# wischmcj/pyQSM

Measured on AMD Instinct MI355X. Metric: Mpoints/s DBSCAN (1M-pt synthetic forest, eps=0.1, min_neighbors=10), higher is better.
Workload: dtype f64; 1 GPU; 1000000-point synthetic tree cloud (configs[1]), DBSCAN eps=0.1 min_neighbors=10, 20 clusters; replicas at N>1; points_per_gpu=1000000, parallelism=replicas x1

## Files before the change

### pyqsm_amd/csrc/dbscan.hip

```cpp
#include "grid.hpp"

#include <atomic>
#include <chrono>
#include <optional>
#include <vector>

namespace pyqsm {

static constexpr int kNoRoot = 0x7FFFFFFF;

__device__ __forceinline__ double sqdist(double ax, double ay, double az, double bx, double by,
                                         double bz) {
  double t0 = ax - bx, t1 = ay - by, t2 = az - bz;
  double d = t0 * t0;
  d = d + t1 * t1;
  d = d + t2 * t2;
  return d;
}


#define FOR_STENCIL(c, st, dir, q, body)                           \
  for (int dz__ = -1; dz__ <= 1; ++dz__)                           \
    for (int dy__ = -1; dy__ <= 1; ++dy__) {                       \
      const int row__ = (c) + dy__ * (st).nx + dz__ * (st).nxy;    \
// ... 75 lines not shown
          const int q = base + lane;
          const int m = qe - base < 64 ? qe - base : 64;
          if (q < qe) co.get(q, L.x[w][lane], L.y[w][lane], L.z[w][lane]);
          __builtin_amdgcn_wave_barrier();
          staged += m;
          if (mine)
            for (int j = 0; j < m; ++j)
              cnt += sqdist(x, y, z, L.x[w][j], L.y[w][j], L.z[w][j]) <= r2;
          __builtin_amdgcn_wave_barrier();
        }
      }
    }
  } else {
#pragma unroll
    for (int ri = 0; ri < 9; ++ri) {
      const int r = kRunOrder[ri];
      for (int base = t.qb[r]; base < t.qe[r] && !deferred; base += 64) {
        const int q = base + lane;
        const int m = t.qe[r] - base < 64 ? t.qe[r] - base : 64;
        if (q < t.qe[r]) co.get(q, L.x[w][lane], L.y[w][lane], L.z[w][lane]);
        __builtin_amdgcn_wave_barrier();
        staged += m;
#pragma unroll 4
        for (int j = 0; j < m; ++j)
          cnt += sqdist(x, y, z, L.x[w][j], L.y[w][j], L.z[w][j]) <= r2;
        __builtin_amdgcn_wave_barrier();
        const unsigned long long und = __ballot(live && cnt < min_pts);
        ++chunks;
        if ((__popcll(und) <= kStragglers || chunks >= max_chunks) &&
            !(ri == 8 && base + 64 >= t.qe[r])) {
          if (und != 0) {
            int slot = 0;
            const int lead = __ffsll(und) - 1;
            const int seg = blockIdx.x % kRestSegs;
            if (lane == lead) slot = atomicAdd(rest_cnt + seg, __popcll(und));
            slot = __shfl(slot, lead, 64);
            if (live && cnt < min_pts) {
              rest[size_t(seg) * seg_cap + slot + __popcll(und & ((1ull << lane) - 1ull))] = p;
              cnt = -1;
            }
          }
          deferred = true;
          break;
        }
      }
    }
  }
  if (live && cnt >= 0) {
    core[p] = cnt >= min_pts;
    co.mark_core(p, cnt >= min_pts);
  }
  if (live) {
    parent[p] = p;
    min_orig[p] = 0x7F7F7F7F;
    flag[p] = 0;
    if (p == n - 1) flag[n] = 0;
  }
  if (tests && lane == 0) atomicAdd(tests + (blockIdx.x & 255), static_cast<unsigned long long>(staged));
  });
}

struct Runs9 {
  int qb[9];
  int pre[10];
  __device__ __forceinline__ int at(int g) const {
    int q = qb[0] + g;
#pragma unroll
    for (int r = 1; r < 9; ++r) q = g >= pre[r] ? qb[r] + (g - pre[r]) : q;
    return q;
  }
};
static constexpr int kRunBatch = 3;
__device__ __forceinline__ int lane_bound(bool act, int c, int j, Stencil st, const CellDir& dir) {
  const int r = int((0x862071534ull >> (4 * (j >> 1))) & 15ull);
  const int cell = c + (r % 3 - 1) * st.nx + (r / 3 - 1) * st.nxy + ((j & 1) ? 2 : -1);
  int b = 0;
  if (act) {
    const DirWord w = dir.words[cell >> 5];
    b = dir.slots[CellDir::slot_of(w, cell)];
  }
  return b;
}
__device__ __forceinline__ Runs9 runs_of_lanes(int bound, int k) {
  Runs9 t;
  t.pre[0] = 0;
#pragma unroll
  for (int r = 0; r < 9; ++r) {
    t.qb[r] = __builtin_amdgcn_readlane(bound, 18 * k + 2 * r);
    t.pre[r + 1] = t.pre[r] + (__builtin_amdgcn_readlane(bound, 18 * k + 2 * r + 1) - t.qb[r]);
  }
  return t;
}

template <class CO>
__global__ __launch_bounds__(256) void k_core_rest(const int32_t* __restrict__ rest,
                                                   const int32_t* __restrict__ rest_cnt ,
                                                   int seg_cap, const GridPlan* __restrict__ plan,
                                                   const DirWord* __restrict__ dwords,
                                                   const int32_t* __restrict__ dslots,
                                                   const int32_t* __restrict__ cell_of, CO co, double r2,
                                                   int min_pts, uint8_t* __restrict__ core,
    unsigned long long* __restrict__ st ) {
  stamped(st, [&] {
  const CellDir dir{dwords, dslots};
  if (!plan->ok) return;
  const Stencil st = plan_stencil(plan);
  const int lane = threadIdx.x & 63;
  const int mine = rest_cnt[lane];
  int incl = mine;
#pragma unroll
  for (int off = 1; off < 64; off <<= 1) {
    const int v = __shfl_up(incl, off, 64);
    if (lane >= off) incl += v;
  }
  const int m = __shfl(incl, 63, 64);
  const int grp = lane / 18, j = lane % 18;
  for (int i0 = (blockIdx.x * 4 + (threadIdx.x >> 6)) * kRunBatch; i0 < m; i0 += gridDim.x * 4 * kRunBatch) {
    int p = 0;
#pragma unroll
    for (int k = 0; k < kRunBatch; ++k) {
      if (i0 + k >= m) break;
      const int seg = __popcll(__ballot(incl <= i0 + k));
      const int before = __shfl(incl - mine, seg, 64);
      const int pk = rest[size_t(seg) * seg_cap + (i0 + k - before)];
      p = grp == k ? pk : p;
    }
    const bool act = grp < kRunBatch && i0 + grp < m;
    double x = 0.0, y = 0.0, z = 0.0;
    int c = 0;
    if (act) {
      co.get(p, x, y, z);
      c = cell_of[p];
    }
    const int bound = lane_bound(act, c, j, st, dir);
#pragma unroll
    for (int k = 0; k < kRunBatch; ++k) {
      if (i0 + k >= m) break;
      const Runs9 t = runs_of_lanes(bound, k);
      const int pk = __builtin_amdgcn_readlane(p, 18 * k);
      const double xk = __shfl(x, 18 * k, 64), yk = __shfl(y, 18 * k, 64), zk = __shfl(z, 18 * k, 64);
      int cnt = 0;
      for (int g0 = 0; g0 < t.pre[9] && cnt < min_pts; g0 += 64) {
        const int g = g0 + lane;
        const bool hit = g < t.pre[9] && co.d2(t.at(g), xk, yk, zk) <= r2;
        cnt += __popcll(__ballot(hit));
      }
      if (lane == 0) {
        core[pk] = cnt >= min_pts;
        co.mark_core(pk, cnt >= min_pts);
      }
    }
  }
  });
}


__device__ __forceinline__ int ld_parent(const int* parent, int i) {
  return __hip_atomic_load(parent + i, __ATOMIC_RELAXED, __HIP_MEMORY_SCOPE_AGENT);
}
__device__ __forceinline__ void st_parent(int* parent, int i, int v) {
  __hip_atomic_store(parent + i, v, __ATOMIC_RELAXED, __HIP_MEMORY_SCOPE_AGENT);
}

__device__ __forceinline__ unsigned link_prio(int x) { return unsigned(x) * 0x9E3779B1u; }

__device__ __forceinline__ int find_root(int* parent, int x) {
  int cur = ld_parent(parent, x);
  if (cur != x) {
    int prev = x, next;
    while (cur != (next = ld_parent(parent, cur))) {
      st_parent(parent, prev, next);
      prev = cur;
      cur = next;
    }
  }
  return cur;
}

__device__ __forceinline__ void unite(int* parent, int a, int b) {
  int ra = find_root(parent, a), rb = find_root(parent, b);
  while (ra != rb) {
    if (link_prio(ra) < link_prio(rb)) {
      int t = ra;
      ra = rb;
      rb = t;
    }
    const int old = atomicCAS(parent + ra, ra, rb);
    if (old == ra) break;
    ra = find_root(parent, old);
    rb = find_root(parent, rb);
  }
}


__global__ __launch_bounds__(1024) void k_sub_rep(int n, const int32_t* __restrict__ sub_of,
                                                 const uint8_t* __restrict__ core,
                                                 const int32_t* __restrict__ order,
                                                 int* __restrict__ parent,
                                                 const int32_t* __restrict__ cell_of,
                                                 int4* __restrict__ rec,
                                                 int* __restrict__ run_min,
                                                 int4* __restrict__ list,
                                                 int32_t* __restrict__ list_cnt, const GridPlan* __restrict__ plan,
                                                 int4* __restrict__ list_xyz,
    unsigned long long* __restrict__ st ) {
  stamped(st, [&] {
  if (!plan->ok) return;
  const int nx = plan->nx, ny = plan->ny;
  const int lane = threadIdx.x & 63, w = threadIdx.x >> 6;
  const int base = blockIdx.x * 1024 + w * 64;
  const int p = base + lane;
  const bool live = p < n;
  int sid = 0, s = n, e = n, ord = 0x7FFFFFFF, cell = 0;
  bool c = false;
  const bool c_prev = base >= 64 && p - 64 < n && core[p - 64];
  const bool c_next = p + 64 < n && core[p + 64];
  const int o_next = c_next ? order[p + 64] : 0x7FFFFFFF;
  if (live) {
    sid = sub_of[p];
    c = core[p];
    if (c) ord = order[p];
    cell = cell_of[p];
    const int2 run = *reinterpret_cast<const int2*>(rec + sid);
    s = run.x;
    e = run.x + run.y;
  }
  const unsigned long long cb = __ballot(c);
  int lead = -1;
  const int s0 = __shfl(s, 0, 64);
  if (s0 < base && s0 >= base - 64) {
    const unsigned long long f = __ballot(c_prev && base - 64 + lane >= s0);
    if (f) lead = base - 64 + __ffsll(f) - 1;
  } else {
    for (int q0 = s0; q0 < base; q0 += 64) {
      const int q = q0 + lane;
      const unsigned long long f = __ballot(q < base && core[q]);
      if (f) {
        lead = q0 + __ffsll(f) - 1;
        break;
      }
    }
  }
  int rep = -1;
  if (c) {
    if (s < base && lead >= 0) {
      rep = lead;
    } else {
      const int lo = s > base ? s - base : 0;
      rep = base + __ffsll(cb & (~0ull << lo)) - 1;
    }
    parent[p] = rep;
  }
  const bool is_rep = c && rep == p;
  int mn = ord;
  const int seg_end = e - base < 64 ? e - base : 64;
#pragma unroll
  for (int off = 1; off < 64; off <<= 1) {
    const int o = __shfl_down(mn, off, 64);
    if (lane + off < seg_end) mn = o < mn ? o : mn;
  }
  const unsigned long long tail = __ballot(is_rep && e > base + 64);
  if (tail) {
    const int t = __ffsll(tail) - 1;
    const int et = __shfl(e, t, 64);
    int m2 = base + 64 + lane < et ? o_next : 0x7FFFFFFF;
    for (int q = base + 128 + lane; q < et; q += 64)
      if (core[q]) m2 = min(m2, order[q]);
#pragma unroll
    for (int off = 32; off > 0; off >>= 1) {
      const int o = __shfl_xor(m2, off, 64);
      m2 = o < m2 ? o : m2;
    }
    if (lane == t) mn = min(mn, m2);
  }
  if (is_rep) {
    rec[sid].z = rep;
    run_min[rep] = mn;
  }
  __shared__ int wcount[16], wbase[16];
  const unsigned long long b = __ballot(is_rep);
  if (lane == 0) wcount[w] = __popcll(b);
  __syncthreads();
  if (threadIdx.x == 0) {
    int tot = 0;
    for (int k = 0; k < 16; ++k) tot += wcount[k];
    int base2 = tot ? atomicAdd(list_cnt, tot) : 0;
    for (int k = 0; k < 16; ++k) {
      wbase[k] = base2;
      base2 += wcount[k];
    }
  }
  __syncthreads();
  if (is_rep) {
    const int slot = wbase[w] + __popcll(b & ((1ull << lane) - 1ull));
    const int c1 = cell;
    list[slot] = make_int4(rep, c1, sid, e - rep);
    list_xyz[slot] = make_int4(c1 % nx, (c1 / nx) % ny, c1 / (nx * ny), sid & 7);
  }
  });
}

__constant__ signed char kSubOffsets[62][3] = {{1,0,0}, {-1,1,0}, {0,1,0}, {1,1,0}, {-1,-1,1}, {0,-1,1}, {1,-1,1}, {-1,0,1}, {0,0,1}, {1,0,1}, {-1,1,1}, {0,1,1}, {1,1,1}, {2,0,0}, {-2,1,0}, {2,1,0}, {-2,2,0}, {-1,2,0}, {0,2,0}, {1,2,0}, {2,2,0}, {-2,-2,1}, {-1,-2,1}, {0,-2,1}, {1,-2,1}, {2,-2,1}, {-2,-1,1}, {2,-1,1}, {-2,0,1}, {2,0,1}, {-2,1,1}, {2,1,1}, {-2,2,1}, {-1,2,1}, {0,2,1}, {1,2,1}, {2,2,1}, {-2,-2,2}, {-1,-2,2}, {0,-2,2}, {1,-2,2}, {2,-2,2}, {-2,-1,2}, {-1,-1,2}, {0,-1,2}, {1,-1,2}, {2,-1,2}, {-2,0,2}, {-1,0,2}, {0,0,2}, {1,0,2}, {2,0,2}, {-2,1,2}, {-1,1,2}, {0,1,2}, {1,1,2}, {2,1,2}, {-2,2,2}, {-1,2,2}, {0,2,2}, {1,2,2}, {2,2,2}};

__global__ __launch_bounds__(256) void k_flatten_reps(const int4* __restrict__ list,
                                                      const int32_t* __restrict__ m_ptr,
                                                      int* __restrict__ parent, int max_steps,
                                                      int4* __restrict__ rec ) {
  const int m = *m_ptr;
  int s = blockIdx.x * 256 + threadIdx.x;
  if (s >= m) return;
  const int4 me = list[s];
  const int p = me.x;
  int r = p, steps = 0;
  for (int nx = parent[r]; nx != r && steps < max_steps; nx = parent[r], ++steps) r = nx;
  parent[p] = r;
  if (rec) {
    int* const word = reinterpret_cast<int*>(rec + (me.z & ~7)) + 3;
    const int old = atomicCAS(word, 0, r + 1);
    if (old != 0 && old != r + 1 && old != -1) *word = -1;
  }
}

static constexpr int kSubPerWave = 4;

struct SubNbr {
  int q0, n2, rep;
};
__device__ __forceinline__ SubNbr sub_neighbour(bool active, const int4 at, int dx, int dy, int dz, int nx, int ny,
                                                const CellDir& dir, const int4* __restrict__ rec) {
  const int gx = 2 * (at.x - 1) + (at.w & 1) - dx, gy = 2 * (at.y - 1) + ((at.w >> 1) & 1) - dy,
            gz = 2 * (at.z - 1) + ((at.w >> 2) & 1) - dz;
  const int c2 = (((gz >> 1) + 1) * ny + ((gy >> 1) + 1)) * nx + ((gx >> 1) + 1);
  const int oct = (gx & 1) | ((gy & 1) << 1) | ((gz & 1) << 2);
  SubNbr out{0, 0, -1};
  DirWord w{0u, 0u};
  if (active) w = dir.words[c2 >> 5];
  if ((w.bits >> (c2 & 31)) & 1u) {
    const int b2 = dir.slots[CellDir::slot_of(w, c2)];
    const int4 r = rec[b2 * 8 + oct];
    if (r.y > 0) {
      out.q0 = r.x;
      out.n2 = r.y;
      out.rep = r.z;
    }
  }
  return out;
}

template <class CO>
__global__ __launch_bounds__(256) void k_hook_sub(const int4* __restrict__ list,
                                                  const int4* __restrict__ list_xyz,
                                                  const int32_t* __restrict__ m_ptr,
                                                  const GridPlan* __restrict__ plan,
                                                  const DirWord* __restrict__ dwords,
                                                  const int32_t* __restrict__ dslots,
                                                  const int4* __restrict__ rec, CO co, double r2,
                                                  const uint8_t* __restrict__ core,
                                                  int* __restrict__ parent,
    unsigned long long* __restrict__ st ) {
  stamped(st, [&] {
  const CellDir dir{dwords, dslots};
  if (!plan->ok) return;
  const int nx = plan->nx, ny = plan->ny;
  const int m = *m_ptr;
  const int k = threadIdx.x & 63;
  const int t = k & 15, grp = k >> 4;
  const int o_dx = t < 13 ? kSubOffsets[t][0] : 0, o_dy = t < 13 ? kSubOffsets[t][1] : 0,
            o_dz = t < 13 ? kSubOffsets[t][2] : 0;
  for (int s0 = (blockIdx.x * 4 + (threadIdx.x >> 6)) * kSubPerWave; s0 < m; s0 += gridDim.x * 4 * kSubPerWave) {
    const bool live = s0 + grp < m;
    const int4 me = list[min(s0 + grp, m - 1)], at = list_xyz[min(s0 + grp, m - 1)];
    const SubNbr nb2 = sub_neighbour(live && t < 13, at, o_dx, o_dy, o_dz, nx, ny, dir, rec);
    const int p = me.x, n1 = me.w;
    unsigned todo = unsigned(__ballot(nb2.rep >= 0) >> (16 * grp)) & 0xFFFFu;
    int base = 0, hooked = -1;
    while (__ballot(todo != 0)) {
      const int src = (k & 48) + (todo ? __ffs(todo) - 1 : 0);
      const int qb = __shfl(nb2.q0, src, 64), nb = __shfl(nb2.n2, src, 64), rb = __shfl(nb2.rep, src, 64);
      const int sh = nb > 1 ? 32 - __clz(nb - 1) : 0;
      const int pairs = n1 << sh;
      const int idx = base + t;
      const int j = idx & ((1 << sh) - 1);
      bool hit = false;
      if (todo && idx < pairs && j < nb) hit = co.core_pair_within(p + (idx >> sh), qb + j, core, r2);
      const bool found = ((__ballot(hit) >> (16 * grp)) & 0xFFFFull) != 0;
      if (found) {
        hooked = rb;
        todo = 0;
      } else if (todo) {
        base += 16;
        if (base >= pairs) {
          todo &= todo - 1;
          base = 0;
        }
      }
    }
    if (hooked >= 0 && t == 0) parent[p] = parent[hooked];
  }
  });
}

template <class CO>
__device__ __forceinline__ bool wave_pair_within(const CO& co, int p, int n1, int qb, int nb, int k,
                                                 const uint8_t* __restrict__ core, double r2) {
  const int sh = nb > 1 ? 32 - __clz(nb - 1) : 0;
  const int pairs = n1 << sh;
  bool found = false;
  for (int base = 0; base < pairs && !found; base += 64) {
    const int idx = base + k;
    const int j = idx & ((1 << sh) - 1);
    bool hit = false;
    if (idx < pairs && j < nb) hit = co.core_pair_within(p + (idx >> sh), qb + j, core, r2);
    found = __ballot(hit) != 0;
  }
  return found;
}

template <class CO>
__device__ __forceinline__ void seam_unite(const int4 me, const int4 at, int k, int o_dx, int o_dy, int o_dz,
                                           int nx, int ny, const CellDir& dir,
                                           const int4* __restrict__ rec, const CO& co, double r2,
                                           const uint8_t* __restrict__ core, int* parent) {
  const SubNbr nb2 = sub_neighbour(k < 62, at, o_dx, o_dy, o_dz, nx, ny, dir, rec);
  const int p = me.x, n1 = me.w, rep2 = nb2.rep;
  const int* vparent = parent;
  int a1 = 0, a2 = 0;
  if (rep2 >= 0) {
    a1 = vparent[p];
    a2 = vparent[rep2];
  }
  bool need = rep2 >= 0 && !(a1 == a2 || a2 == p || a1 == rep2);
  int root2 = -1;
  if (need) {
    int ra = a1, rb = a2;
    for (;;) {
      const int pa = ld_parent(parent, ra), pb = ld_parent(parent, rb);
      if (pa == ra && pb == rb) break;
      ra = pa;
      rb = pb;
    }
    need = ra != rb;
    root2 = rb;
  }
  unsigned long long todo = __ballot(need);
  while (todo) {
    const int src = __ffsll(todo) - 1;
    todo &= todo - 1;
    const int qb = __shfl(nb2.q0, src, 64), nb = __shfl(nb2.n2, src, 64), rb = __shfl(rep2, src, 64);
    const int tree = __shfl(root2, src, 64);
    if (wave_pair_within(co, p, n1, qb, nb, k, core, r2)) {
      if (k == 0) unite(parent, p, rb);
      todo &= ~__ballot(root2 == tree);
    }
  }
}

template <class CO>
__global__ __launch_bounds__(256) void k_union_sub(const int4* __restrict__ list,
                                                   const int4* __restrict__ list_xyz,
                                                   const int32_t* __restrict__ m_ptr,
                                                   const GridPlan* __restrict__ plan,
                                                   const DirWord* __restrict__ dwords,
                                                   const int32_t* __restrict__ dslots,
                                                   const int4* __restrict__ rec, CO co, double r2,
                                                   const uint8_t* __restrict__ core, int* parent,
                                                   unsigned long long* __restrict__ seam_cnt ,
    unsigned long long* __restrict__ st ) {
  stamped(st, [&] {
  const CellDir dir{dwords, dslots};
  if (!plan->ok) return;
  const int nx = plan->nx, ny = plan->ny;
  const int m = *m_ptr;
  const int k = threadIdx.x & 63;
  const int t = k & 15, grp = k >> 4;
  const int o_dx = k < 62 ? kSubOffsets[k][0] : 0, o_dy = k < 62 ? kSubOffsets[k][1] : 0,
            o_dz = k < 62 ? kSubOffsets[k][2] : 0;
  const int c_off = t < 9 ? (t % 3 - 1) + (t / 3 - 1) * nx : 0;
  const int layer = nx * ny;
  for (int s0 = (blockIdx.x * 4 + (threadIdx.x >> 6)) * kSubPerWave; s0 < m; s0 += gridDim.x * 4 * kSubPerWave) {
    const bool live = s0 + grp < m;
    const int4 me = list[min(s0 + grp, m - 1)];
    const int* vparent = parent;
    const int r_s = vparent[me.x];
    const int c2 = me.y + c_off;
    int word[2] = {0, 0};
    DirWord dw[2] = {{0u, 0u}, {0u, 0u}};
    if (live && t < 9) {
#pragma unroll
      for (int l = 0; l < 2; ++l) dw[l] = dir.words[(c2 - l * layer) >> 5];
    }
    int b2[2] = {0, 0};
    bool occ[2];
#pragma unroll
    for (int l = 0; l < 2; ++l) {
      occ[l] = (dw[l].bits >> ((c2 - l * layer) & 31)) & 1u;
      if (occ[l]) b2[l] = dir.slots[CellDir::slot_of(dw[l], c2 - l * layer)];
    }
#pragma unroll
    for (int l = 0; l < 2; ++l)
      if (occ[l]) word[l] = rec[b2[l] * 8].w;
    const unsigned long long seams =
        __ballot((word[0] != 0 && word[0] != r_s + 1) || (word[1] != 0 && word[1] != r_s + 1));
    if (!seams) continue;
    for (int u = 0; u < kSubPerWave; ++u) {
      if (!((seams >> (16 * u)) & 0xFFFFull)) continue;
      if (seam_cnt && k == 0) atomicAdd(seam_cnt, 1ull);
      seam_unite(list[s0 + u], list_xyz[s0 + u], k, o_dx, o_dy, o_dz, nx, ny, dir, rec, co, r2, core, parent);
    }
  }
  });
}

template <class CO>
__global__ __launch_bounds__(256) void k_union_points(int n, Stencil st,
                                                      const DirWord* __restrict__ dwords,
                                                      const int32_t* __restrict__ dslots,
                                                      const int32_t* __restrict__ cell_of, CO co, double r2,
                                                      const uint8_t* __restrict__ core, int* parent) {
  const CellDir dir{dwords, dslots};
  int p = blockIdx.x * 256 + threadIdx.x;
  if (p >= n || !core[p]) return;
  double x, y, z;
  co.get(p, x, y, z);
  const int c = cell_of[p];
  const volatile int* vparent = parent;
  int rp = find_root(parent, p);
  FOR_STENCIL(c, st, dir, q, {
    if (q < p && core[q] && co.d2(q, x, y, z) <= r2) {
      if (vparent[q] != rp) {
        unite(parent, p, q);
        rp = find_root(parent, p);
      }
    }
  })
}

__global__ __launch_bounds__(256) void k_flatten(int n, const uint8_t* __restrict__ core,
                                                 int* __restrict__ parent, const GridPlan* __restrict__ plan) {
  int p = blockIdx.x * 256 + threadIdx.x;
  if (!plan->ok || p >= n || !core[p]) return;
  int r = p;
  for (int nx = parent[r]; nx != r; nx = parent[r]) r = nx;
  parent[p] = r;
}

template <int kThreads>
__device__ __forceinline__ void block_append(bool take, int value, int32_t* __restrict__ list,
                                             int32_t* __restrict__ cnt) {
  constexpr int kWaves = kThreads / 64;
  __shared__ int wcount[kWaves], wbase[kWaves];
  const unsigned long long b = __ballot(take);
  const int lane = threadIdx.x & 63, w = threadIdx.x >> 6;
  if (lane == 0) wcount[w] = __popcll(b);
  __syncthreads();
  if (threadIdx.x == 0) {
    int tot = 0;
    for (int k = 0; k < kWaves; ++k) tot += wcount[k];
    int base = tot ? atomicAdd(cnt, tot) : 0;
    for (int k = 0; k < kWaves; ++k) {
      wbase[k] = base;
      base += wcount[k];
    }
  }
  __syncthreads();
  if (take) list[wbase[w] + __popcll(b & ((1ull << lane) - 1ull))] = value;
}

static constexpr int kFlagsThreads = 256, kFlagsPer = 16, kFlagsPerBlock = kFlagsThreads * kFlagsPer;
__device__ __forceinline__ void flags_role(int b, int n, const uint8_t* __restrict__ core,
                                           int32_t* __restrict__ rest, int32_t* __restrict__ rest_cnt) {
  constexpr int kWaves = kFlagsThreads / 64;
  __shared__ int fcount[kWaves], fbase[kWaves];
  const int lane = threadIdx.x & 63, w = threadIdx.x >> 6;
  const int p0 = b * kFlagsPerBlock + threadIdx.x;
  unsigned take = 0;
#pragma unroll
  for (int k = 0; k < kFlagsPer; ++k) {
    const int p = p0 + k * kFlagsThreads;
    take |= unsigned(p < n && !core[p]) << k;
  }
  int mine = __popc(take);
#pragma unroll
  for (int off = 32; off > 0; off >>= 1) mine += __shfl_xor(mine, off, 64);
  if (lane == 0) fcount[w] = mine;
  __syncthreads();
  if (threadIdx.x == 0) {
    int tot = 0;
    for (int k = 0; k < kWaves; ++k) tot += fcount[k];
    int base = tot ? atomicAdd(rest_cnt, tot) : 0;
    for (int k = 0; k < kWaves; ++k) {
      fbase[k] = base;
      base += fcount[k];
    }
  }
  __syncthreads();
  int at = fbase[w];
#pragma unroll
  for (int k = 0; k < kFlagsPer; ++k) {
    const bool t = (take >> k) & 1u;
    const unsigned long long bal = __ballot(t);
    if (t) rest[at + __popcll(bal & ((1ull << lane) - 1ull))] = p0 + k * kFlagsThreads;
    at += __popcll(bal);
  }
}

__global__ __launch_bounds__(kFlagsThreads) void k_noncore_list(int n, const uint8_t* __restrict__ core,
                                                                int32_t* __restrict__ rest,
                                                                int32_t* __restrict__ rest_cnt,
                                                                const GridPlan* __restrict__ plan) {
  if (!plan->ok) return;
  flags_role(blockIdx.x, n, core, rest, rest_cnt);
}

__global__ __launch_bounds__(256) void k_point_min(int n, const uint8_t* __restrict__ core,
                                                   const int* __restrict__ parent,
                                                   const int32_t* __restrict__ order,
                                                   int* __restrict__ min_orig,
                                                   int32_t* __restrict__ roots,
                                                   int32_t* __restrict__ roots_cnt,
                                                   const GridPlan* __restrict__ plan) {
  int p = blockIdx.x * 256 + threadIdx.x;
  const bool is_c = plan->ok && p < n && core[p];
  if (is_c) atomicMin(min_orig + parent[p], order[p]);
  block_append<256>(is_c && parent[p] == p, p, roots, roots_cnt);
}

static constexpr int kRepRootThreads = kFlagsThreads;
static_assert(kRepRootThreads == 256, "gl, the grid of the representatives' blocks, is cut in 256s");
__global__ __launch_bounds__(kRepRootThreads) void k_rep_root(const int4* __restrict__ list,
                                                  const int32_t* __restrict__ m_ptr,
                                                  int* __restrict__ parent,
                                                  const int* __restrict__ run_min,
                                                  int* __restrict__ min_orig,
                                                  int32_t* __restrict__ roots,
                                                  int32_t* __restrict__ roots_cnt, int rep_blocks, int n,
                                                  const uint8_t* __restrict__ core, int32_t* __restrict__ rest,
                                                  int32_t* __restrict__ rest_cnt,
                                                  const GridPlan* __restrict__ plan) {
  if (int(blockIdx.x) >= rep_blocks) {
    if (plan->ok) flags_role(blockIdx.x - rep_blocks, n, core, rest, rest_cnt);
    return;
  }
  const int m = *m_ptr;
  int s = blockIdx.x * kRepRootThreads + threadIdx.x;
  const bool active = s < m;
  int p = -1, r = -1, v = 0x7FFFFFFF;
  if (active) {
    p = list[s].x;
    r = p;
    for (int nx = parent[r]; nx != r; nx = parent[r]) r = nx;
    if (r != p) parent[p] = r;
    v = run_min[p];
  }
  const volatile int* vmin = min_orig;
  const int lane = threadIdx.x & 63;
  unsigned long long rem = __ballot(active);
  while (rem) {
    const int lead = __ffsll(rem) - 1;
    const int r0 = __shfl(r, lead, 64);
    const bool mine = active && r == r0;
    int mn = mine ? v : 0x7FFFFFFF;
#pragma unroll
    for (int off = 32; off > 0; off >>= 1) {
      const int o = __shfl_xor(mn, off, 64);
      mn = o < mn ? o : mn;
    }
    if (lane == lead && mn < vmin[r0]) atomicMin(min_orig + r0, mn);
    rem &= ~__ballot(mine);
  }
  block_append<256>(active && r == p, p, roots, roots_cnt);
}

static constexpr int kRankCap = 4096;
static constexpr int kNumberThreads = 1024;

__global__ __launch_bounds__(kNumberThreads) void k_number(int n, const int32_t* __restrict__ roots,
                                                           const int32_t* __restrict__ roots_cnt,
                                                           int* __restrict__ min_orig,
                                                           uint32_t* __restrict__ bits ,
                                                           int32_t* __restrict__ wpre ,
                                                           int32_t* __restrict__ done ,
                                                           const GridPlan* __restrict__ plan,
    unsigned long long* __restrict__ st ) {
  stamped(st, [&] {
  if (!plan->ok) return;
  const int R = *roots_cnt;
  const int t = threadIdx.x;
  if (R <= kRankCap) {
    if (blockIdx.x != 0) return;
    __shared__ unsigned long long key[kRankCap];
    int P = 2;
    while (P < R) P <<= 1;
    for (int i = t; i < P; i += kNumberThreads) {
      unsigned long long k = ~0ull;
      if (i < R) {
        const int r = roots[i];
        k = (static_cast<unsigned long long>(min_orig[r]) << 32) | static_cast<uint32_t>(r);
      }
      key[i] = k;
    }
    __syncthreads();
    for (int k = 2; k <= P; k <<= 1)
      for (int j = k >> 1; j > 0; j >>= 1) {
        for (int i = t; i < P; i += kNumberThreads) {
          const int l = i ^ j;
          if (l > i) {
            const unsigned long long a = key[i], b = key[l];
            if ((a > b) == ((i & k) == 0)) {
              key[i] = b;
              key[l] = a;
            }
          }
        }
        __syncthreads();
      }
    for (int i = t; i < R; i += kNumberThreads) min_orig[static_cast<uint32_t>(key[i])] = i;
    return;
  }
  for (int i = blockIdx.x * kNumberThreads + t; i < R; i += gridDim.x * kNumberThreads) {
    const int v = min_orig[roots[i]];
    __hip_atomic_fetch_or(bits + (v >> 5), 1u << (v & 31), __ATOMIC_RELAXED, __HIP_MEMORY_SCOPE_AGENT);
  }
  __shared__ int last;
  __threadfence();
  __syncthreads();
  if (t == 0) last = atomicAdd(done, 1) == int(gridDim.x) - 1;
  __syncthreads();
  if (!last) return;
  __threadfence();
  __shared__ int wsum[kNumberThreads / 64];
  const int lane = t & 63, wv = t >> 6;
  const int nw = n / 32 + 1;
  int carry = 0;
  for (int w0 = 0; w0 < nw; w0 += 16 * kNumberThreads) {
    const int i0 = w0 + 16 * t;
    int cnt[16], sum = 0;
#pragma unroll
    for (int k = 0; k < 16; ++k) {
      cnt[k] = i0 + k < nw ? __popc(__hip_atomic_load(bits + i0 + k, __ATOMIC_RELAXED, __HIP_MEMORY_SCOPE_AGENT)) : 0;
      sum += cnt[k];
    }
    int incl = sum;
#pragma unroll
    for (int off = 1; off < 64; off <<= 1) {
      const int o = __shfl_up(incl, off, 64);
      if (lane >= off) incl += o;
    }
    if (lane == 63) wsum[wv] = incl;
    __syncthreads();
    int before = carry, total = 0;
    for (int k = 0; k < kNumberThreads / 64; ++k) {
      before += k < wv ? wsum[k] : 0;
      total += wsum[k];
    }
    int run = before + incl - sum;
#pragma unroll
    for (int k = 0; k < 16; ++k)
      if (i0 + k < nw) {
        wpre[i0 + k] = run;
        run += cnt[k];
      }
    carry += total;
    __syncthreads();
  }
  });
}

__device__ __forceinline__ int cluster_number(int v, int n_roots, const uint32_t* __restrict__ bits,
                                              const int32_t* __restrict__ wpre) {
  if (n_roots <= kRankCap) return v;
  return wpre[v >> 5] + __popc(bits[v >> 5] & ((1u << (v & 31)) - 1u));
}

static constexpr int kLabelThreads = 256;
template <class CO>
__global__ __launch_bounds__(kLabelThreads) void k_labels(int n, const int32_t* __restrict__ rest,
                                                          const int32_t* __restrict__ rest_cnt,
                                                          const GridPlan* __restrict__ plan,
                                                          const DirWord* __restrict__ dwords,
                                                          const int32_t* __restrict__ dslots,
                                                          const int32_t* __restrict__ cell_of, CO co, double r2,
                                                          const uint8_t* __restrict__ core,
                                                          const int* __restrict__ parent,
                                                          const int* __restrict__ min_orig,
                                                          const int32_t* __restrict__ roots_cnt,
                                                          const uint32_t* __restrict__ bits,
                                                          const int32_t* __restrict__ wpre,
                                                          const int32_t* __restrict__ order,
                                                          int64_t* __restrict__ labels,
                                                          uint8_t* __restrict__ is_core,
    unsigned long long* __restrict__ st ) {
  stamped(st, [&] {
  const CellDir dir{dwords, dslots};
  if (!plan->ok) return;
  constexpr int kWaves = kLabelThreads / 64;
  const int n_roots = *roots_cnt;
  const int lane = threadIdx.x & 63;
  {
    const int p = blockIdx.x * kLabelThreads + threadIdx.x;
    const bool is_c = p < n && core[p];
    if (is_c) {
      const int v = min_orig[parent[parent[p]]];
      labels[order[p]] = int64_t(cluster_number(v, n_roots, bits, wpre));
    }
    if (p < n && is_core) is_core[order[p]] = is_c;
  }
  const int m = *rest_cnt;
  const Stencil sten = plan_stencil(plan);
  const int first = (blockIdx.x * kWaves + __builtin_amdgcn_readfirstlane(threadIdx.x >> 6)) * kRunBatch;
  const int grp = lane / 18, j = lane % 18;
  for (int i0 = first; i0 < m; i0 += gridDim.x * kWaves * kRunBatch) {
    const bool act = grp < kRunBatch && i0 + grp < m;
    double x = 0.0, y = 0.0, z = 0.0;
    int p = 0, c = 0;
    if (act) {
      p = rest[i0 + grp];
      co.get(p, x, y, z);
      c = cell_of[p];
    }
    const int bound = lane_bound(act, c, j, sten, dir);
#pragma unroll
    for (int k = 0; k < kRunBatch; ++k) {
      if (i0 + k >= m) break;
      const Runs9 t = runs_of_lanes(bound, k);
      const int pk = __builtin_amdgcn_readlane(p, 18 * k);
      const double xk = __shfl(x, 18 * k, 64), yk = __shfl(y, 18 * k, 64), zk = __shfl(z, 18 * k, 64);
      int best = kNoRoot;
      for (int g0 = 0; g0 < t.pre[9]; g0 += 64) {
        const int g = g0 + lane;
        if (g < t.pre[9]) {
          const int q = t.at(g);
          if (core[q] && co.d2(q, xk, yk, zk) <= r2) {
            const int mo = min_orig[parent[parent[q]]];
            best = mo < best ? mo : best;
          }
        }
      }
#pragma unroll
      for (int off = 32; off > 0; off >>= 1) {
        const int o = __shfl_xor(best, off, 64);
        best = o < best ? o : best;
      }
      if (lane == 0)
        labels[order[pk]] = best == kNoRoot ? int64_t(-1) : int64_t(cluster_number(best, n_roots, bits, wpre));
    }
  }
  });
}

static int cluster_binned(Ctx* c, int64_t n, double eps, int32_t min_pts, bool radius_inclusive, const DevGrid& g,
                          const SubCells& sub, const GridPlan* d_plan, int64_t* labels, uint8_t* is_core,
                          const int32_t** count_out) {
  const bool fine = g.cell <= eps * (1.0 + 1.0 / 524288.0);
  const int N = int(n);
  const dim3 grid(ceil_div(n, 256)), block(256);
  const Stencil st{g.nx, g.nx * g.ny};
  const CellDir dir = cell_dir(g);
  const double r2 = radius_inclusive ? eps * eps : nextafter(eps * eps, 0.0);
  uint8_t* core;
  int *parent, *min_orig;
  int32_t* flag;
  PQ_TRY(c->arena.get(size_t(n), &core));
  PQ_TRY(c->arena.get(size_t(n), &parent));
  PQ_TRY(c->arena.get(size_t(n), &min_orig));
  PQ_TRY(c->arena.get(size_t(n) + 1, &flag));
  uint32_t* const bits = reinterpret_cast<uint32_t*>(flag);
  int32_t *roots, *wpre;
  PQ_TRY(c->arena.get(size_t(n), &roots));
  PQ_TRY(c->arena.get(size_t(n / 32) + 1, &wpre));
  int4* list;
  int32_t* list_cnt;
  int* run_min;
  PQ_TRY(c->arena.get(size_t(n), &run_min));
  PQ_TRY(c->arena.get(size_t(n), &list));
  int4* list_xyz;
  PQ_TRY(c->arena.get(size_t(n), &list_xyz));
  list_cnt = sub.zeroed4;
  int32_t* const roots_cnt = list_cnt + 1;
  int32_t* rest;
  const int core_blocks = int(ceil_div(n, 256));
  const int seg_cap = ceil_div(core_blocks, kRestSegs) * 256;
  PQ_TRY(c->arena.get(std::max<size_t>(size_t(n), size_t(seg_cap) * kRestSegs), &rest));
  int32_t* const rest_segs = list_cnt + 4;
  {
    StampScope ps(c, "dbscan_core");
    unsigned long long* d_tests = nullptr;
    if (c->prof >= 2) {
      PQ_TRY(c->arena.get(256, &d_tests));
      PQ_HIP(hipMemsetAsync(d_tests, 0, 256 * 8, c->stream));
    }
    const int max_chunks = std::min(32, std::max(kMaxChunks, (kMaxChunks * min_pts + 9) / 10));
    {
      const StampKernel pk(c, "k_core_tiled", grid.x);
      on_coords(g, [&](auto co) {
        hipLaunchKernelGGL(k_core_tiled<decltype(co)>, grid, block, 0, c->stream, N, d_plan, dir.words, dir.slots, g.cell_of, co, r2,
                           min_pts, core, rest, rest_segs, seg_cap, parent, min_orig, flag, max_chunks, d_tests,
                           pk.slots);
      });
    }
    if (d_tests) {
      unsigned long long h[256];
      PQ_HIP(hipMemcpyAsync(h, d_tests, sizeof(h), hipMemcpyDeviceToHost, c->stream));
      PQ_HIP(hipStreamSynchronize(c->stream));
      unsigned long long tot = 0;
      for (unsigned long long v : h) tot += v;
      c->timers["core_pair_tests"].launches += int64_t(tot) * 64;
    }
    const dim3 gr(std::min<int64_t>(8192, ceil_div(n, 64)));
    unsigned long long* const st_rest = stamp_slots(c, gr.x);
    on_coords(g, [&](auto co) {
      hipLaunchKernelGGL(k_core_rest<decltype(co)>, gr, block, 0, c->stream, rest, rest_segs, seg_cap, d_plan, dir.words, dir.slots,
                         g.cell_of, co, r2, min_pts, core, st_rest);
    });
    PQ_HIP(hipGetLastError());
    if (getenv("PYQSM_DBSCAN_TRACE")) {
      int32_t h[kRestSegs];
      PQ_HIP(hipMemcpyAsync(h, rest_segs, sizeof(h), hipMemcpyDeviceToHost, c->stream));
      PQ_HIP(hipStreamSynchronize(c->stream));
      long long tot = 0;
      for (int32_t v : h) tot += v;
      fprintf(stderr, "core pass: %lld stragglers\n", tot);
    }
  }
  {
    StampScope ps(c, "dbscan_union");
    const dim3 gf(ceil_div(n, kFlagsPerBlock));
    if (fine) {
      hipLaunchKernelGGL(k_sub_rep, dim3(ceil_div(n, 1024)), dim3(1024), 0, c->stream, N, sub.sub_of, core,
                         g.order, parent, g.cell_of, sub.rec, run_min, list, list_cnt, d_plan, list_xyz,
                         stamp_slots(c, ceil_div(n, 1024)));
      {
        int per_cu[2] = {16, 32};
        if (const char* e_cu = getenv("PYQSM_UNION_BLOCKS_PER_CU")) {
          per_cu[0] = per_cu[1] = atoi(e_cu);
          if (const char* comma = strchr(e_cu, ',')) per_cu[1] = atoi(comma + 1);
        }
        const int64_t full = ceil_div(n, 4 * kSubPerWave);
        const dim3 gh(per_cu[0] > 0 ? std::min<int64_t>(full, int64_t(c->cu_count) * per_cu[0]) : full),
            gu(per_cu[1] > 0 ? std::min<int64_t>(full, int64_t(c->cu_count) * per_cu[1]) : full),
            gl(ceil_div(n, 256));
        const bool trace = getenv("PYQSM_DBSCAN_TRACE") != nullptr;
        {
          const StampKernel pk(c, "k_hook_sub", gh.x);
          on_coords(g, [&](auto co) {
            hipLaunchKernelGGL(k_hook_sub<decltype(co)>, gh, block, 0, c->stream, list, list_xyz, list_cnt, d_plan,
                               dir.words, dir.slots, sub.rec, co, r2, core, parent, pk.slots);
          });
        }
        if (trace) {
          int32_t m = 0;
          PQ_HIP(hipMemcpyAsync(&m, list_cnt, 4, hipMemcpyDeviceToHost, c->stream));
          PQ_HIP(hipStreamSynchronize(c->stream));
          std::vector<int32_t> hp(static_cast<size_t>(n), 0);
          std::vector<int4> hl(static_cast<size_t>(m), make_int4(0, 0, 0, 0));
          PQ_HIP(hipMemcpy(hp.data(), parent, size_t(n) * 4, hipMemcpyDeviceToHost));
          PQ_HIP(hipMemcpy(hl.data(), list, size_t(m) * 16, hipMemcpyDeviceToHost));
          std::vector<int64_t> hist(66, 0);
          int64_t roots = 0;
          for (int32_t s2 = 0; s2 < m; ++s2) {
            int d = 0, r = hl[size_t(s2)].x;
            while (hp[size_t(r)] != r && d < 65) {
              r = hp[size_t(r)];
              ++d;
            }
            hist[size_t(d)]++;
            roots += d == 0;
          }
          fprintf(stderr, "hook pass: %d sub-cells, %lld roots; chain depth histogram:", m, (long long)roots);
          for (int d = 0; d < 66; ++d)
            if (hist[size_t(d)]) fprintf(stderr, " %d:%lld", d, (long long)hist[size_t(d)]);
          fprintf(stderr, "\n");
        }
        static const int jump = [] {
          const char* e = getenv("PYQSM_FLATTEN_JUMP");
          return e ? atoi(e) : 12;
        }();
        if (jump > 0)
          hipLaunchKernelGGL(k_flatten_reps, gl, block, 0, c->stream, list, list_cnt, parent, jump,
                             static_cast<int4*>(nullptr));
        hipLaunchKernelGGL(k_flatten_reps, gl, block, 0, c->stream, list, list_cnt, parent, 0x7fffffff, sub.rec);
        unsigned long long* d_seams = nullptr;
        if (trace) {
          PQ_TRY(c->arena.get(1, &d_seams));
          PQ_HIP(hipMemsetAsync(d_seams, 0, 8, c->stream));
        }
        {
          const StampKernel pk(c, "k_union_sub", gu.x);
          on_coords(g, [&](auto co) {
            hipLaunchKernelGGL(k_union_sub<decltype(co)>, gu, block, 0, c->stream, list, list_xyz, list_cnt, d_plan,
                               dir.words, dir.slots, sub.rec, co, r2, core, parent, d_seams, pk.slots);
          });
        }
        if (trace) {
          unsigned long long h = 0;
          PQ_HIP(hipMemcpyAsync(&h, d_seams, 8, hipMemcpyDeviceToHost, c->stream));
          PQ_HIP(hipStreamSynchronize(c->stream));
          fprintf(stderr, "seam union: %llu sub-cells took the 62-offset path\n", h);
        }
        hipLaunchKernelGGL(k_rep_root, dim3(gl.x + gf.x), dim3(kRepRootThreads), 0, c->stream, list, list_cnt, parent,
                           run_min, min_orig, roots, roots_cnt, int(gl.x), N, core, rest, list_cnt + 3, d_plan);
      }
      PQ_HIP(hipGetLastError());
    } else {
      PQ_TRY(stamp_mark(c));
      on_coords(g, [&](auto co) {
        hipLaunchKernelGGL(k_union_points<decltype(co)>, grid, block, 0, c->stream, N, st, dir.words, dir.slots, g.cell_of, co,
                           r2, core, parent);
      });
      hipLaunchKernelGGL(k_flatten, grid, block, 0, c->stream, N, core, parent, d_plan);
      hipLaunchKernelGGL(k_point_min, grid, block, 0, c->stream, N, core, parent, g.order, min_orig, roots,
                         roots_cnt, d_plan);
      hipLaunchKernelGGL(k_noncore_list, gf, dim3(kFlagsThreads), 0, c->stream, N, core, rest,
                         list_cnt + 3, d_plan);
    }
    const dim3 gn(std::min<int64_t>(ceil_div(n, kNumberThreads), c->cu_count));
    hipLaunchKernelGGL(k_number, gn, dim3(kNumberThreads), 0, c->stream, N, roots, roots_cnt, min_orig, bits, wpre,
                       list_cnt + 2, d_plan, stamp_slots(c, gn.x));
    PQ_HIP(hipGetLastError());
  }
  {
    StampScope ps(c, "dbscan_label");
    const dim3 gb(ceil_div(n, kLabelThreads));
    unsigned long long* const st_labels = stamp_slots(c, gb.x);
    on_coords(g, [&](auto co) {
      hipLaunchKernelGGL(k_labels<decltype(co)>, gb, dim3(kLabelThreads), 0, c->stream, N, rest, list_cnt + 3, d_plan,
                         dir.words, dir.slots, g.cell_of, co, r2, core, parent, min_orig, roots_cnt, bits, wpre, g.order, labels,
                         is_core, st_labels);
    });
    PQ_HIP(hipGetLastError());
    if (getenv("PYQSM_DBSCAN_TRACE")) {
      int32_t h = 0;
      PQ_HIP(hipMemcpyAsync(&h, list_cnt + 3, 4, hipMemcpyDeviceToHost, c->stream));
      PQ_HIP(hipStreamSynchronize(c->stream));
      fprintf(stderr, "label pass: %d non-core points listed\n", h);
    }
  }
  *count_out = roots_cnt;
  return 0;
}


static constexpr double kPlanPollMs = 20.0;
static int wait_plan(Ctx* c, const GridPlan* h_plan, unsigned seq) {
  const volatile unsigned* const s = &h_plan->seq;
  const auto t0 = std::chrono::steady_clock::now();
  while (*s != seq) {
    if (std::chrono::duration<double, std::milli>(std::chrono::steady_clock::now() - t0).count() > kPlanPollMs) {
      PQ_HIP(hipStreamSynchronize(c->stream));
      if (*s != seq) return fail(PYQSM_EHIP, "DBSCAN: the grid plan was not written (sequence %u)", seq);
      break;
    }
  }
  std::atomic_thread_fence(std::memory_order_acquire);
  return 0;
}

struct DirReadout {
  int64_t cap;
  int32_t* begin_host;
  int32_t dims[3];
};
static int dbscan_device(Ctx* c, const double* xyz, int64_t n, double eps, int32_t min_pts,
                         bool radius_inclusive, int64_t* labels, uint8_t* is_core, int64_t* n_clusters,
                         DirReadout* readout = nullptr) {
  if (!(eps > 0) || !std::isfinite(eps)) return fail(PYQSM_EINVAL, "eps must be positive");
  if (n == 0) {
    if (n_clusters) *n_clusters = 0;
    return 0;
  }
  const double cell = eps * (1.0 + 1.0 / 1048576.0);
  const int64_t max_cells = int64_t(1) << 28;
  if (!c->plan_pinned) {
    PQ_HIP(hipHostMalloc(&c->plan_pinned, 2 * sizeof(GridPlan), hipHostMallocMapped | hipHostMallocCoherent));
    memset(c->plan_pinned, 0, 2 * sizeof(GridPlan));
  }
  GridPlan* const h_plan = static_cast<GridPlan*>(c->plan_pinned);
  GridPlan* h_plan_dev;
  PQ_HIP(hipHostGetDevicePointer(reinterpret_cast<void**>(&h_plan_dev), c->plan_pinned, 0));
  if (++c->plan_seq == 0) c->plan_seq = 1;
  const unsigned seq = c->plan_seq;
  GridPlan* d_plan;
  int32_t* zeroed;
  PQ_TRY(c->arena.get(2, &d_plan));
  PQ_TRY(c->arena.get(size_t(octant_zeroed_ints()), &zeroed));
  const char* plan_env = getenv("PYQSM_DBSCAN_PLAN");
  const char* bin_env = getenv("PYQSM_DBSCAN_BIN");
  const char* f32_env = getenv("PYQSM_COORD_F32");
  const bool speculate = c->plan_hint.valid && !(plan_env && !strcmp(plan_env, "host")) && !bin_env &&
                         !(f32_env && !strcmp(f32_env, "0")) && n <= (int64_t(1) << 25);
  const PlanHint hint = speculate ? c->plan_hint : PlanHint{};
  DevGrid g;
  SubCells sub;
  const int32_t* count = nullptr;
  std::optional<StampScope> bin_scope(std::in_place, c, "dbscan_bin");
  PQ_TRY(plan_grid_device(c, xyz, n, cell, max_cells, hint, d_plan, h_plan_dev, seq, zeroed, octant_zeroed_ints()));
  const Arena::Mark mark = c->arena.mark();
  if (speculate) {
    PQ_TRY(bin_octants_planned(c, xyz, n, cell, hint, d_plan, zeroed, &g, &sub));
    bin_scope.reset();
    if (!readout)
      PQ_TRY(cluster_binned(c, n, eps, min_pts, radius_inclusive, g, sub, d_plan, labels, is_core, &count));
  }
  PQ_TRY(wait_plan(c, h_plan, seq));
  const bool hit = speculate && h_plan[0].ok;
  if (!hit) {
    c->arena.rewind(mark);
    PlanHint next;
    if (!bin_scope) bin_scope.emplace(c, "dbscan_bin");
    PQ_TRY(stamp_mark(c));
    PQ_TRY(bin_octants_host(c, xyz, n, cell, max_cells, h_plan[0], zeroed, &h_plan[1], d_plan + 1, &g, &sub, &next));
    PQ_TRY(stamp_mark(c));
    bin_scope.reset();
    if (next.valid) c->plan_hint = next;
    if (!readout)
      PQ_TRY(cluster_binned(c, n, eps, min_pts, radius_inclusive, g, sub, d_plan + 1, labels, is_core, &count));
  }
  if (c->prof >= 1) {
    c->timers["dbscan_f32_records"].launches += g.p4 ? 1 : 0;
    c->timers[hit ? "dbscan_plan_hit" : "dbscan_plan_miss"].launches += 1;
  }
  if (readout) {
    const GridPlan& pl = hit ? h_plan[0] : h_plan[1];
    readout->dims[0] = pl.nx;
    readout->dims[1] = pl.ny;
    readout->dims[2] = pl.nz;
    const int64_t entries = int64_t(pl.ncell) + 1;
    if (entries > readout->cap)
      return fail(PYQSM_ERANGE, "octant directory: %lld entries, room for %lld", (long long)entries,
                  (long long)readout->cap);
    int32_t* d_begin;
    PQ_TRY(c->arena.get(size_t(entries), &d_begin));
    read_directory(c, g, pl.ncell, d_begin);
    PQ_HIP(hipGetLastError());
    PQ_HIP(hipMemcpyAsync(readout->begin_host, d_begin, size_t(entries) * 4, hipMemcpyDeviceToHost, c->stream));
    PQ_HIP(hipStreamSynchronize(c->stream));
    return 0;
  }
  if (n_clusters) {
    int32_t h = 0;
    PQ_HIP(hipMemcpyAsync(&h, count, 4, hipMemcpyDeviceToHost, c->stream));
    PQ_HIP(hipStreamSynchronize(c->stream));
    *n_clusters = h;
  }
  return 0;
}

}

using namespace pyqsm;

extern "C" {

int pyqsm_dbscan_dev_ex(const double* xyz_dev, int64_t n, double eps, int32_t min_pts,
                        int32_t radius_inclusive, int64_t* labels_dev, uint8_t* is_core_dev,
                        int64_t* n_clusters, int32_t device) {
  PQ_API_RANGE("pyqsm_dbscan_dev");
  if (n < 0) return fail(PYQSM_EINVAL, "negative size");
  if (n > 0 && (!xyz_dev || !labels_dev)) return fail(PYQSM_EINVAL, "pyqsm_dbscan_dev: NULL pointer");
  Ctx* c = ctx_for(device);
  if (!c) return PYQSM_ENODEV;
  std::lock_guard<std::mutex> lk(c->mu);
  c->arena.reset();
  StampScope ps(c, "dbscan_total");
  return dbscan_device(c, xyz_dev, n, eps, min_pts, radius_inclusive != 0, labels_dev, is_core_dev,
                       n_clusters);
}

int pyqsm_dbscan_dev(const double* xyz_dev, int64_t n, double eps, int32_t min_pts,
                     int64_t* labels_dev, uint8_t* is_core_dev, int64_t* n_clusters,
                     int32_t device) {
  return pyqsm_dbscan_dev_ex(xyz_dev, n, eps, min_pts, 1, labels_dev, is_core_dev, n_clusters, device);
}

int pyqsm_dbscan(const double* xyz, int64_t n, double eps, int32_t min_pts, int64_t* labels,
                 uint8_t* is_core, int32_t device) {
  return pyqsm_dbscan_ex(xyz, n, eps, min_pts, 1, labels, is_core, device);
}

int pyqsm_dbscan_ex(const double* xyz, int64_t n, double eps, int32_t min_pts, int32_t radius_inclusive,
                    int64_t* labels, uint8_t* is_core, int32_t device) {
  PQ_API_RANGE("pyqsm_dbscan");
  if (n < 0) return fail(PYQSM_EINVAL, "negative size");
  if (n == 0) return 0;
  if (!xyz || !labels) return fail(PYQSM_EINVAL, "pyqsm_dbscan: NULL pointer");
  Ctx* c = ctx_for(device);
  if (!c) return PYQSM_ENODEV;
  std::lock_guard<std::mutex> lk(c->mu);
  c->arena.reset();
  double* d_xyz;
  int64_t* d_lab;
  uint8_t* d_core;
  PQ_TRY(c->arena.get(size_t(n) * 3, &d_xyz));
  PQ_TRY(c->arena.get(size_t(n), &d_lab));
  PQ_TRY(c->arena.get(size_t(n), &d_core));
  PQ_HIP(hipMemcpyAsync(d_xyz, xyz, size_t(n) * 24, hipMemcpyHostToDevice, c->stream));
  PQ_TRY(dbscan_device(c, d_xyz, n, eps, min_pts, radius_inclusive != 0, d_lab, d_core, nullptr));
  PQ_HIP(hipMemcpyAsync(labels, d_lab, size_t(n) * 8, hipMemcpyDeviceToHost, c->stream));
  if (is_core) PQ_HIP(hipMemcpyAsync(is_core, d_core, size_t(n), hipMemcpyDeviceToHost, c->stream));
  PQ_HIP(hipStreamSynchronize(c->stream));
  return 0;
}

int pyqsm_octant_directory(const double* xyz, int64_t n, double eps, int32_t* dims_out, int32_t* begin_out,
                           int64_t cap, int32_t device) {
  PQ_API_RANGE("pyqsm_octant_directory");
  if (n <= 0) return fail(PYQSM_EINVAL, "pyqsm_octant_directory: empty cloud");
  if (!xyz || !dims_out || !begin_out) return fail(PYQSM_EINVAL, "pyqsm_octant_directory: NULL pointer");
  Ctx* c = ctx_for(device);
  if (!c) return PYQSM_ENODEV;
  std::lock_guard<std::mutex> lk(c->mu);
  c->arena.reset();
  double* d_xyz;
  PQ_TRY(c->arena.get(size_t(n) * 3, &d_xyz));
  PQ_HIP(hipMemcpyAsync(d_xyz, xyz, size_t(n) * 24, hipMemcpyHostToDevice, c->stream));
  DirReadout ro{cap, begin_out, {0, 0, 0}};
  PQ_TRY(dbscan_device(c, d_xyz, n, eps, 1, true, nullptr, nullptr, nullptr, &ro));
  for (int a = 0; a < 3; ++a) dims_out[a] = ro.dims[a];
  return 0;
}

}
```

Baseline: 3257 Mpoints/s.

## Record second hook link per sub-cell and unite it in a flatten pass

```diff
diff --git a/pyqsm_amd/csrc/dbscan.hip b/pyqsm_amd/csrc/dbscan.hip
--- a/pyqsm_amd/csrc/dbscan.hip
+++ b/pyqsm_amd/csrc/dbscan.hip
@@ -401,22 +401,53 @@
 
 __constant__ signed char kSubOffsets[62][3] = {{1,0,0}, {-1,1,0}, {0,1,0}, {1,1,0}, {-1,-1,1}, {0,-1,1}, {1,-1,1}, {-1,0,1}, {0,0,1}, {1,0,1}, {-1,1,1}, {0,1,1}, {1,1,1}, {2,0,0}, {-2,1,0}, {2,1,0}, {-2,2,0}, {-1,2,0}, {0,2,0}, {1,2,0}, {2,2,0}, {-2,-2,1}, {-1,-2,1}, {0,-2,1}, {1,-2,1}, {2,-2,1}, {-2,-1,1}, {2,-1,1}, {-2,0,1}, {2,0,1}, {-2,1,1}, {2,1,1}, {-2,2,1}, {-1,2,1}, {0,2,1}, {1,2,1}, {2,2,1}, {-2,-2,2}, {-1,-2,2}, {0,-2,2}, {1,-2,2}, {2,-2,2}, {-2,-1,2}, {-1,-1,2}, {0,-1,2}, {1,-1,2}, {2,-1,2}, {-2,0,2}, {-1,0,2}, {0,0,2}, {1,0,2}, {2,0,2}, {-2,1,2}, {-1,1,2}, {0,1,2}, {1,1,2}, {2,1,2}, {-2,2,2}, {-1,2,2}, {0,2,2}, {1,2,2}, {2,2,2}};
 
+enum FlattenMode { kFlattenJump, kFlattenRoots, kFlattenLink, kFlattenWords };
+
+template <FlattenMode MODE>
 __global__ __launch_bounds__(256) void k_flatten_reps(const int4* __restrict__ list,
                                                       const int32_t* __restrict__ m_ptr,
-                                                      int* __restrict__ parent, int max_steps,
+                                                      int* parent, int max_steps ,
+                                                      const int32_t* __restrict__ link2 ,
                                                       int4* __restrict__ rec ) {
   const int m = *m_ptr;
-  int s = blockIdx.x * 256 + threadIdx.x;
-  if (s >= m) return;
-  const int4 me = list[s];
-  const int p = me.x;
-  int r = p, steps = 0;
-  for (int nx = parent[r]; nx != r && steps < max_steps; nx = parent[r], ++steps) r = nx;
-  parent[p] = r;
-  if (rec) {
-    int* const word = reinterpret_cast<int*>(rec + (me.z & ~7)) + 3;
-    const int old = atomicCAS(word, 0, r + 1);
-    if (old != 0 && old != r + 1 && old != -1) *word = -1;
+  const int s = blockIdx.x * 256 + threadIdx.x;
+  const bool active = s < m;
+  if constexpr (MODE == kFlattenJump || MODE == kFlattenLink) {
+    if (!active) return;
+  }
+  int p = -1, r = -1, cell8 = -1;
+  if (active) {
+    const int4 me = list[s];
+    p = r = me.x;
+    cell8 = me.z & ~7;
+  }
+  if constexpr (MODE == kFlattenJump) {
+    int steps = 0;
+    for (int nx = parent[r]; nx != r && steps < max_steps; nx = parent[r], ++steps) r = nx;
+    if (r != p) parent[p] = r;
+  } else if constexpr (MODE == kFlattenLink) {
+    const int l = link2[s];
+    int r2 = l >= 0 ? l : p;
+    for (;;) {
+      const int a = parent[r], b = parent[r2];
+      if (a == r && b == r2) break;
+      r = a;
+      r2 = b;
+    }
+    if (r != p) parent[p] = r;
+    if (r2 != r) unite(parent, r, r2);
+  } else {
+    if (active) {
+      for (int nx = parent[r]; nx != r; nx = parent[r]) r = nx;
+      if (r != p) parent[p] = r;
+    }
+    const int pc = __shfl_up(cell8, 1, 64), pr = __shfl_up(r, 1, 64);
+    const bool dup = (threadIdx.x & 63) != 0 && pc == cell8 && pr == r;
+    if (active && !dup) {
+      int* const word = reinterpret_cast<int*>(rec + cell8) + 3;
+      const int old = atomicCAS(word, 0, r + 1);
+      if (old != 0 && old != r + 1 && old != -1) *word = -1;
+    }
   }
 }
 
@@ -446,7 +477,7 @@
   return out;
 }
 
-template <class CO>
+template <class CO, bool LINK2>
 __global__ __launch_bounds__(256) void k_hook_sub(const int4* __restrict__ list,
                                                   const int4* __restrict__ list_xyz,
                                                   const int32_t* __restrict__ m_ptr,
@@ -456,6 +487,7 @@
                                                   const int4* __restrict__ rec, CO co, double r2,
                                                   const uint8_t* __restrict__ core,
                                                   int* __restrict__ parent,
+                                                  int32_t* __restrict__ link2 ,
     unsigned long long* __restrict__ st ) {
   stamped(st, [&] {
   const CellDir dir{dwords, dslots};
@@ -472,7 +504,7 @@
     const SubNbr nb2 = sub_neighbour(live && t < 13, at, o_dx, o_dy, o_dz, nx, ny, dir, rec);
     const int p = me.x, n1 = me.w;
     unsigned todo = unsigned(__ballot(nb2.rep >= 0) >> (16 * grp)) & 0xFFFFu;
-    int base = 0, hooked = -1;
+    int base = 0, hooked = -1, second = -1;
     while (__ballot(todo != 0)) {
       const int src = (k & 48) + (todo ? __ffs(todo) - 1 : 0);
       const int qb = __shfl(nb2.q0, src, 64), nb = __shfl(nb2.n2, src, 64), rb = __shfl(nb2.rep, src, 64);
@@ -484,8 +516,14 @@
       if (todo && idx < pairs && j < nb) hit = co.core_pair_within(p + (idx >> sh), qb + j, core, r2);
       const bool found = ((__ballot(hit) >> (16 * grp)) & 0xFFFFull) != 0;
       if (found) {
-        hooked = rb;
-        todo = 0;
+        if (LINK2 && hooked < 0) {
+          hooked = rb;
+          todo &= todo - 1;
+          base = 0;
+        } else {
+          if (LINK2) second = rb; else hooked = rb;
+          todo = 0;
+        }
       } else if (todo) {
         base += 16;
         if (base >= pairs) {
@@ -495,6 +533,7 @@
       }
     }
     if (hooked >= 0 && t == 0) parent[p] = parent[hooked];
+    if (LINK2 && live && t == 0) link2[s0 + grp] = second;
   }
   });
 }
@@ -974,6 +1013,8 @@
   PQ_TRY(c->arena.get(size_t(n), &list));
   int4* list_xyz;
   PQ_TRY(c->arena.get(size_t(n), &list_xyz));
+  int32_t* link2;
+  PQ_TRY(c->arena.get(size_t(n), &link2));
   list_cnt = sub.zeroed4;
   int32_t* const roots_cnt = list_cnt + 1;
   int32_t* rest;
@@ -1029,7 +1070,11 @@
                          g.order, parent, g.cell_of, sub.rec, run_min, list, list_cnt, d_plan, list_xyz,
                          stamp_slots(c, ceil_div(n, 1024)));
       {
-        int per_cu[2] = {16, 32};
+        static const bool use_link2 = [] {
+          const char* e = getenv("PYQSM_DBSCAN_LINK2");
+          return e ? atoi(e) != 0 : true;
+        }();
+        int per_cu[2] = {use_link2 ? 8 : 16, 32};
         if (const char* e_cu = getenv("PYQSM_UNION_BLOCKS_PER_CU")) {
           per_cu[0] = per_cu[1] = atoi(e_cu);
           if (const char* comma = strchr(e_cu, ',')) per_cu[1] = atoi(comma + 1);
@@ -1042,42 +1087,80 @@
         {
           const StampKernel pk(c, "k_hook_sub", gh.x);
           on_coords(g, [&](auto co) {
-            hipLaunchKernelGGL(k_hook_sub<decltype(co)>, gh, block, 0, c->stream, list, list_xyz, list_cnt, d_plan,
-                               dir.words, dir.slots, sub.rec, co, r2, core, parent, pk.slots);
+            if (use_link2)
+              hipLaunchKernelGGL((k_hook_sub<decltype(co), true>), gh, block, 0, c->stream, list, list_xyz, list_cnt,
+                                 d_plan, dir.words, dir.slots, sub.rec, co, r2, core, parent, link2, pk.slots);
+            else
+              hipLaunchKernelGGL((k_hook_sub<decltype(co), false>), gh, block, 0, c->stream, list, list_xyz, list_cnt,
+                                 d_plan, dir.words, dir.slots, sub.rec, co, r2, core, parent, link2, pk.slots);
           });
         }
-        if (trace) {
-          int32_t m = 0;
-          PQ_HIP(hipMemcpyAsync(&m, list_cnt, 4, hipMemcpyDeviceToHost, c->stream));
+        int32_t tm = 0;
+        std::vector<int32_t> hp, root_of;
+        std::vector<int4> hl;
+        const auto snapshot = [&](std::vector<int64_t>* hist) -> int {
+          PQ_HIP(hipMemcpyAsync(&tm, list_cnt, 4, hipMemcpyDeviceToHost, c->stream));
           PQ_HIP(hipStreamSynchronize(c->stream));
-          std::vector<int32_t> hp(static_cast<size_t>(n), 0);
-          std::vector<int4> hl(static_cast<size_t>(m), make_int4(0, 0, 0, 0));
+          hp.assign(static_cast<size_t>(n), 0);
+          hl.assign(static_cast<size_t>(tm), make_int4(0, 0, 0, 0));
           PQ_HIP(hipMemcpy(hp.data(), parent, size_t(n) * 4, hipMemcpyDeviceToHost));
-          PQ_HIP(hipMemcpy(hl.data(), list, size_t(m) * 16, hipMemcpyDeviceToHost));
-          std::vector<int64_t> hist(66, 0);
-          int64_t roots = 0;
-          for (int32_t s2 = 0; s2 < m; ++s2) {
+          PQ_HIP(hipMemcpy(hl.data(), list, size_t(tm) * 16, hipMemcpyDeviceToHost));
+          root_of.assign(static_cast<size_t>(n), -1);
+          for (int32_t s2 = 0; s2 < tm; ++s2) {
             int d = 0, r = hl[size_t(s2)].x;
-            while (hp[size_t(r)] != r && d < 65) {
+            while (hp[size_t(r)] != r) {
               r = hp[size_t(r)];
               ++d;
             }
-            hist[size_t(d)]++;
-            roots += d == 0;
+            root_of[size_t(hl[size_t(s2)].x)] = r;
+            if (hist) (*hist)[size_t(std::min(d, 65))]++;
           }
-          fprintf(stderr, "hook pass: %d sub-cells, %lld roots; chain depth histogram:", m, (long long)roots);
+          return 0;
+        };
+        const auto count_roots = [&] {
+          int64_t roots = 0;
+          for (int32_t s2 = 0; s2 < tm; ++s2) roots += root_of[size_t(hl[size_t(s2)].x)] == hl[size_t(s2)].x;
+          return roots;
+        };
+        int64_t links = 0, crossing = 0;
+        if (trace) {
+          std::vector<int64_t> hist(66, 0);
+          PQ_TRY(snapshot(&hist));
+          fprintf(stderr, "hook pass: %d sub-cells, %lld roots; chain depth histogram:", tm, (long long)count_roots());
           for (int d = 0; d < 66; ++d)
             if (hist[size_t(d)]) fprintf(stderr, " %d:%lld", d, (long long)hist[size_t(d)]);
           fprintf(stderr, "\n");
+          if (use_link2) {
+            std::vector<int32_t> h2(static_cast<size_t>(tm), -1);
+            PQ_HIP(hipMemcpy(h2.data(), link2, size_t(tm) * 4, hipMemcpyDeviceToHost));
+            for (int32_t s2 = 0; s2 < tm; ++s2) {
+              if (h2[size_t(s2)] < 0) continue;
+              ++links;
+              crossing += root_of[size_t(h2[size_t(s2)])] != root_of[size_t(hl[size_t(s2)].x)];
+            }
+          }
         }
         static const int jump = [] {
           const char* e = getenv("PYQSM_FLATTEN_JUMP");
           return e ? atoi(e) : 12;
         }();
         if (jump > 0)
-          hipLaunchKernelGGL(k_flatten_reps, gl, block, 0, c->stream, list, list_cnt, parent, jump,
-                             static_cast<int4*>(nullptr));
-        hipLaunchKernelGGL(k_flatten_reps, gl, block, 0, c->stream, list, list_cnt, parent, 0x7fffffff, sub.rec);
+          hipLaunchKernelGGL(k_flatten_reps<kFlattenJump>, gl, block, 0, c->stream, list, list_cnt, parent, jump,
+                             link2, sub.rec);
+        if (use_link2) {
+          hipLaunchKernelGGL(k_flatten_reps<kFlattenLink>, gl, block, 0, c->stream, list, list_cnt, parent, 0, link2,
+                             sub.rec);
+          if (trace) {
+            PQ_TRY(snapshot(nullptr));
+            fprintf(stderr, "link pass: %lld recorded, %lld crossed trees, %lld roots left\n", (long long)links,
+                    (long long)crossing, (long long)count_roots());
+          }
+          hipLaunchKernelGGL(k_flatten_reps<kFlattenWords>, gl, block, 0, c->stream, list, list_cnt, parent, 0, link2,
+                             sub.rec);
+        } else {
+          hipLaunchKernelGGL(k_flatten_reps<kFlattenRoots>, gl, block, 0, c->stream, list, list_cnt, parent, 0, link2,
+                             sub.rec);
+        }
         unsigned long long* d_seams = nullptr;
         if (trace) {
           PQ_TRY(c->arena.get(1, &d_seams));
```

Measured after the change: 3425 Mpoints/s (median of 6 runs). 1.05x the previous value.
